# zipnn/zipnn

Measured on AMD Instinct MI355X. Metric: bf16 decompress GB/s (uncompressed bytes / s; compress GB/s beside it), higher is better.
Workload: dtype u8; 1 GPU; 4 GiB synthetic bf16 N(0,0.02) tensor per GPU, 256 KiB chunks, byte-split + huff0 (BASELINE.json configs[1]); chunks_per_gpu=16384, parallelism=chunk-sharded x1, no collectives

## Files before the change

### zipnn_amd/csrc/zn_decode_fused.hip

```cpp
#include "zn_internal.hpp"
#include <atomic>
#include "zn_huf_wave.hpp"
#include "zn_decode_common.hpp"
#include "zn_decode_rest.hpp"

#define ZN_F_THREADS 256
#define ZN_F_RING_BYTES 4096u
#define ZN_F_WAVES_PER_SIMD 4
#define ZN_F_RING_DW (ZN_F_RING_BYTES / 4u)
#define ZN_F_DMAX 6
#define ZN_F_DCAP 4
#define ZN_F_DOM_MAX 154
#define ZN_F_DCONST 4
#define ZN_F_DCONST2 6
#define ZN_F_DENSE_LMIN 4
#define ZN_F_IN_DW (64 * ZN_F_DMAX + 4)
#define ZN_F_TF(D) ((D) * 4 + 1)
#define ZN_F_TLMAX 11u
#define ZN_L16(i) ((i) + (((i) >> 6) << 1))
#define ZN_F_PRIO_SYNC 1
#define ZN_F_PRIO_COUNT 2
#define ZN_F_PRIO_WRITE 3
#if !defined(ZN_SIMT_EMULATOR)
#define ZN_PRIO(v) __builtin_amdgcn_s_setprio(v)
#else
#define ZN_PRIO(v) do { } while (0)
#endif
#if !defined(ZN_SIMT_EMULATOR)
#define ZN_OPAQUE32(x) asm volatile("" : "+v"(x))
#define ZN_KEEP32(x) asm volatile("" :: "v"(x))
__device__ __forceinline__ uint32_t zn_bfi_(uint32_t mask, uint32_t a, uint32_t b) {
  uint32_t d; asm("v_bfi_b32 %0, %1, %2, %3" : "=v"(d) : "s"(mask), "v"(a), "v"(b)); return d;
}
#define ZN_BFI(mask, a, b) zn_bfi_((mask), (a), (b))
#define ZN_NO_IFCVT asm volatile("")
#define ZN_ASM_MARK(txt) asm volatile("; " txt)
#else
#define ZN_NO_IFCVT ((void)0)
#define ZN_ASM_MARK(txt) ((void)0)
#define ZN_OPAQUE32(x) ((void)0)
#define ZN_KEEP32(x) ((void)(x))
#define ZN_BFI(mask, a, b) ((((uint32_t)(a)) & (uint32_t)(mask)) | (((uint32_t)(b)) & ~(uint32_t)(mask)))
#endif
#define ZN_F_DELTA0 44
#define ZN_F_DELTA0_DENSE 88
#define ZN_F_DELTA_FAST 44
#define ZN_F_DELTA_MAX 1024
#define ZN_F_NMIS 3

#if defined(ZN_SIMT_EMULATOR) && defined(ZN_DECODE_HINTED_TU)
extern unsigned long long zn_dbg_tiles[8], zn_dbg_hint[4];
#define ZN_DBG_COUNT(i) do { if (lane == 0) zn_dbg_tiles[i]++; } while (0)
#define ZN_HINT_COUNT(i, n) do { if (lane == 0) zn_dbg_hint[i] += (n); } while (0)
#define ZN_HINT_FIXUP() do { if (hinted && !hfix) { hfix = true; ZN_HINT_COUNT(1, 1); } } while (0)
#elif defined(ZN_SIMT_EMULATOR)
unsigned long long zn_dbg_tiles[8];
extern "C" void zn_debug_tile_counters(unsigned long long* out, int reset) { for (int i = 0; i < 8; i++) { out[i] = zn_dbg_tiles[i]; if (reset) zn_dbg_tiles[i] = 0; } }
#define ZN_DBG_COUNT(i) do { if (lane == 0) zn_dbg_tiles[i]++; } while (0)
unsigned long long zn_dbg_hint[4];
extern "C" void zn_debug_hint_counters(unsigned long long* out, int reset) { for (int i = 0; i < 4; i++) { out[i] = zn_dbg_hint[i]; if (reset) zn_dbg_hint[i] = 0; } }
#define ZN_HINT_COUNT(i, n) do { if (lane == 0) zn_dbg_hint[i] += (n); } while (0)
#define ZN_HINT_FIXUP() do { if (hinted && !hfix) { hfix = true; ZN_HINT_COUNT(1, 1); } } while (0)
#else
#define ZN_DBG_COUNT(i) do { } while (0)
#define ZN_HINT_COUNT(i, n) do { } while (0)
#define ZN_HINT_FIXUP() do { } while (0)
#endif

#define ZN_IN_IDX(i) (i)

#if !defined(ZN_SIMT_EMULATOR)
typedef uint32_t zn_v4u __attribute__((ext_vector_type(4)));
#define ZN_ST128(p, a, b, c, d) __builtin_nontemporal_store((zn_v4u){(a), (b), (c), (d)}, (zn_v4u*)(p))
#else
#define ZN_ST128(p, a, b, c, d) (*(uint4*)(p) = make_uint4((a), (b), (c), (d)))
#endif

#if defined(ZN_SIMT_EMULATOR)
__device__ __forceinline__ uint32_t zn_lane_id() { return threadIdx.x & 63u; }
#else
__device__ __forceinline__ uint32_t zn_lane_id() { return __builtin_amdgcn_mbcnt_hi(~0u, __builtin_amdgcn_mbcnt_lo(~0u, 0u)); }
#endif
__device__ __forceinline__ uint32_t zn_uniform(uint32_t v) { return (uint32_t)__builtin_amdgcn_readfirstlane((int)v); }
__device__ __forceinline__ uint64_t zn_uniform64(uint64_t v) { return ((uint64_t)zn_uniform((uint32_t)(v >> 32)) << 32) | zn_uniform((uint32_t)v); }
template <typename T> __device__ __forceinline__ T* zn_uniform_ptr(T* p) { return ZN_GLOBAL_PTR(T, zn_uniform64((uint64_t)p)); }

typedef uint64_t __attribute__((aligned(1))) zn_u64u;
typedef uint32_t __attribute__((aligned(1))) zn_u32u;
#if !defined(ZN_SIMT_EMULATOR)
#define ZN_LD_RAW32(p) __builtin_nontemporal_load((const zn_u32u*)(p))
#define ZN_LD_RAW64(p) __builtin_nontemporal_load((const zn_u64u*)(p))
#define ZN_LD_STREAM32(p) __builtin_nontemporal_load((const uint32_t*)(p))
#else
#define ZN_LD_RAW32(p) (*(const zn_u32u*)(p))
#define ZN_LD_RAW64(p) (*(const zn_u64u*)(p))
#define ZN_LD_STREAM32(p) (*(const uint32_t*)(p))
#endif
#if defined(ZN_SIMT_EMULATOR)
#define ZN_ST128_4(p, a, b, c, d) (*(uint4*)(p) = make_uint4((a), (b), (c), (d)))
#else
#define ZN_ST128_4(p, a, b, c, d) ZN_ST128(p, a, b, c, d)
#endif

__device__ __forceinline__ uint64_t zn_hint_header_bytes(uint64_t pk) { return ((pk + 1u) * 4u + 63u) & ~63ull; }
__device__ __forceinline__ uint32_t zn_hint_stream_bytes(uint32_t slen, uint32_t seg, uint32_t unit) {
  uint32_t d = ((ZN_F_RING_BYTES - unit - 128u) * slen) / (256u * seg);
  d = d > ZN_F_DCAP ? ZN_F_DCAP : (d < 1u ? 1u : d);
  const uint32_t dw = (slen + 6u) >> 2, td = 64u * d;
  return 64u * ((dw + td - 1u) / td);
}

struct ZnFusedPlane { uint64_t off; uint32_t kind; uint32_t csize; };

struct __attribute__((aligned(16))) ZnFusedLds {
  uint2 lut[1u << ZN_F_TLMAX];
  uint32_t ring[4][ZN_F_RING_DW];
  uint32_t in[4][ZN_F_IN_DW];
  uint8_t symlist[4][256];
  uint32_t rank_start[4][14], sym_start[4][14];
  ZnFusedPlane plane[4][4];
  ZnWaveStats st[4];
  uint32_t what[4];
};

#include "zn_decode_chain.hpp"

template <int NT = ZN_F_THREADS, typename LDS>
__device__ __forceinline__ void zn_fused_fill_luts(LDS& L, uint32_t tid, uint32_t TL, uint32_t j, uint32_t lmin = 1) {
  constexpr int KE = (int)((1u << ZN_F_TLMAX) / (uint32_t)NT);
  uint16_t* lut16 = (uint16_t*)&L.ring[0][0];
  {
    const ZnRankTab rt = zn_load_ranks(L.rank_start[j], L.sym_start[j]);
    for (uint32_t u = tid; u < (1u << TL); u += (uint32_t)NT) lut16[ZN_L16(u)] = (uint16_t)zn_lut_entry(u, TL, L.symlist[j], rt, L.rank_start[j], L.sym_start[j]);
  }
  __syncthreads();
  {
    const uint32_t mask = (1u << TL) - 1u;
    uint32_t pos[KE], cnt[KE], syms[KE], ef[KE];
    for (int k = 0; k < KE; k++) { pos[k] = 0; cnt[k] = 0; syms[k] = 0; ef[k] = 0; }
    const int rounds = (int)zn_uniform(lmin ? (TL / lmin > 4u ? 4u : TL / lmin) : 4u);
    for (int step = 0; step < 4; step++) {
      if (step >= rounds) break;
      for (int k = 0; k < KE; k++) {
        const uint32_t u = tid + (uint32_t)k * (uint32_t)NT;
        if (u <= mask && cnt[k] == (uint32_t)step) {
          const uint32_t e = lut16[ZN_L16((u << pos[k]) & mask)]; const uint32_t len = e >> 8;
          if (pos[k] + len <= TL) {
            if (step > 0) ef[k] |= pos[k] << (16 + 4 * (step - 1));
            syms[k] |= (e & 0xFFu) << (8 * step);
            pos[k] += len; cnt[k]++;
          }
        }
      }
    }
    for (int k = 0; k < KE; k++) {
      const uint32_t u = tid + (uint32_t)k * (uint32_t)NT;
      for (uint32_t i = 1; i <= 3u; i++) if (i >= cnt[k]) ef[k] |= pos[k] << (16u + 4u * (i - 1u));
      if (u <= mask) L.lut[u] = make_uint2(syms[k], ZN_E_META(cnt[k], pos[k], ef[k]));
    }
  }
}

template <int P, int H, int DC, bool X = false, int HM = 0>
__device__ __forceinline__ bool zn_fused_wave(const ZnGeom& g, const uint8_t* __restrict__ body, const uint8_t* body_end,
                                              uint8_t* outq_, const uint8_t* xq_, const ZnFusedPlane (&pl_)[P], const uint8_t* const (&rawq_)[P],
                                              const uint2* lut, uint32_t* ring, uint32_t* in, uint32_t lane_, uint32_t seg_,
                                              uint32_t TL_, uint32_t Du, const uint8_t* stream_, uint32_t slen_, bool ragged ZN_PT_PARAM,
                                              uint8_t* hq_ = nullptr, uint32_t hcap_ = 0) {
  uint32_t lane = lane_;
  uint8_t* const outq = zn_uniform_ptr(outq_); const uint8_t* const xq = zn_uniform_ptr(xq_);
  const uint8_t* const stream = zn_uniform_ptr(stream_);
  const uint32_t seg = zn_uniform(seg_), TL = zn_uniform(TL_), slen = zn_uniform(slen_);
  ZnFusedPlane pl[P]; const uint8_t* rawq[P];
  for (int p = 0; p < P; p++) {
    pl[p].off = zn_uniform64(pl_[p].off); pl[p].kind = zn_uniform(pl_[p].kind); pl[p].csize = zn_uniform(pl_[p].csize);
    rawq[p] = zn_uniform_ptr(rawq_[p]);
  }
  constexpr int EPL = (P == 1) ? 16 : 8;
  constexpr int EW = EPL / 4;
  constexpr uint32_t UNIT = 64u * EPL;
  uint8_t* const hq = HM ? zn_uniform_ptr(hq_) : nullptr; const uint32_t hcap = HM ? zn_uniform(hcap_) : 0u;
  const bool hinted = (HM == 1) && hq != nullptr;
  uint32_t ht = 0, hb_nx = 0;
#define ZN_F_RB4 2
#define ZN_F_SPLIT4 1
  constexpr bool SPLIT = (P == 4) && (ZN_F_SPLIT4 != 0);
#define ZN_F_RB2 3
  constexpr int RB = (P == 2) ? (int)ZN_F_RB2 : (P == 4) ? ZN_F_RB4 : (int)(ZN_F_RING_BYTES / 1024u);
  constexpr int TF = DC ? ZN_F_TF(DC) : 0, TB = 3;
  constexpr bool DENSE = (ZN_F_DCONST2 != 0) && (DC == ZN_F_DCONST2);
  constexpr int UF = DC ? (32 * DC - 31) / 11 : 0;
  ZN_PT_SHARED;

  uint32_t pre[RB][P][EW];
  uint32_t lane_v = lane;
  auto fetch_row_to = [&](uint32_t (&pre)[RB][P][EW], uint32_t first_row_sym, int r) {
    if constexpr (HM == 2) return;
    for (int p = 0; p < P; p++) if (p != H && pl[p].kind == ZN_KIND_RAW) {
      const uint8_t* au = rawq[p] + (first_row_sym + (uint32_t)r * UNIT);
      if constexpr (SPLIT) {
        const uint8_t* a = au + 4u * lane_v;
        pre[r][p][0] = ZN_LD_RAW32(a); pre[r][p][1 % EW] = ZN_LD_RAW32(a + UNIT / 2u);
      } else {
        const uint8_t* a = au + (uint32_t)EPL * lane_v;
        for (int k = 0; k < EW / 2; k++) { const uint64_t t = ZN_LD_RAW64(a + 8 * k); pre[r][p][2 * k] = (uint32_t)t; pre[r][p][2 * k + 1] = (uint32_t)(t >> 32); }
      }
    }
  };
  auto fetch_row = [&](uint32_t first_row_sym, int r) { fetch_row_to(pre, first_row_sym, r); };
  auto fetch_rows = [&](uint32_t first_row_sym, int nrows) {
    for (int r = 0; r < RB; r++) if (r < nrows) fetch_row_to(pre, first_row_sym, r);
  };
  auto emit_rows_from = [&](uint32_t (&pre)[RB][P][EW], bool full_wait, uint32_t first_row_sym, int nrows, uint32_t stage_row0, auto&& after_wait) {
    if (full_wait) __builtin_amdgcn_s_waitcnt(0x0F70);
    ZN_PT(10);
    after_wait();
    constexpr int XW = X ? (P == 4 ? 8 : 4) : 1, XG = 2;
    uint32_t xd[2][XG][XW];
    auto load_delta = [&](int grp) {
      for (int i = 0; i < XG; i++) {
        const int r = grp * XG + i;
        for (int k = 0; k < XW; k++) xd[grp & 1][i][k] = 0;
        if (xq && r < RB && r < nrows) {
          const uint8_t* a = SPLIT ? xq + (uint64_t)(first_row_sym + (uint32_t)r * UNIT) * P + 16u * lane
                                   : xq + (uint64_t)(first_row_sym + (uint32_t)r * UNIT + (uint32_t)EPL * lane) * P;
          for (int k = 0; k < XW / 4; k++) { const uint4 t = *(const uint4*)(a + (SPLIT ? (UNIT / 2u) * P : 16u) * k); xd[grp & 1][i][4 * k] = t.x; xd[grp & 1][i][4 * k + 1] = t.y; xd[grp & 1][i][4 * k + 2] = t.z; xd[grp & 1][i][4 * k + 3] = t.w; }
        }
      }
    };
    if (X) load_delta(0);
    for (int r = 0; r < RB; r++) if (r < nrows) {
      for (int p = 0; p < P; p++) {
        if (p == H) {
          if constexpr (SPLIT) { const uint32_t i = ((stage_row0 + (uint32_t)r) * UNIT >> 2) + lane; for (int k = 0; k < EW; k++) { pre[r][p][k] = ring[i + (UNIT / 8u) * k]; ring[i + (UNIT / 8u) * k] = 0; } }
          else { const uint32_t i = ((stage_row0 + (uint32_t)r) * UNIT + (uint32_t)EPL * lane) >> 2; for (int k = 0; k < EW; k++) { pre[r][p][k] = ring[i + k]; ring[i + k] = 0; } }
        }
        else if (pl[p].kind == ZN_KIND_RLE) { ZN_NO_IFCVT; for (int k = 0; k < EW; k++) pre[r][p][k] = ((uint32_t)pl[p].off & 0xFFu) * 0x01010101u; }
      }
    }
    if (P >= 2 && g.rot) {
      for (int r = 0; r < RB; r++) if (r < nrows)
        for (int k = 0; k < EW; k++) {
          const uint32_t hi = pre[r][P - 1][k], lo = pre[r][(P >= 2) ? P - 2 : 0][k];
          pre[r][P - 1][k] = ZN_BFI(0x80808080u, lo, hi >> 1);
          pre[r][(P >= 2) ? P - 2 : 0][k] = ZN_BFI(0x7F7F7F7Fu, lo, hi << 7);
        }
    }
    if constexpr (HM != 2)
    for (int r = 0; r < RB; r++) if (r < nrows) {
      if (X && r % XG == 0 && r + XG < RB) load_delta(r / XG + 1);
      const uint32_t* xr_ = xd[(r / XG) & 1][r % XG];
      uint8_t* o = (outq + (uint64_t)(first_row_sym + (uint32_t)r * UNIT) * P) + (SPLIT ? 16u : (uint32_t)EPL * (uint32_t)P) * lane_v;
      if (P == 1) {
        if (X) ZN_ST128(o, pre[r][0][0] ^ xr_[0], pre[r][0][1 % EW] ^ xr_[1 % XW], pre[r][0][2 % EW] ^ xr_[2 % XW], pre[r][0][3 % EW] ^ xr_[3 % XW]);
        else ZN_ST128(o, pre[r][0][0], pre[r][0][1 % EW], pre[r][0][2 % EW], pre[r][0][3 % EW]);
      } else if (P == 2) {
        uint32_t x[4];
        x[0] = __builtin_amdgcn_perm(pre[r][1 % P][0], pre[r][0][0], 0x05010400u); x[1] = __builtin_amdgcn_perm(pre[r][1 % P][0], pre[r][0][0], 0x07030602u);
        x[2] = __builtin_amdgcn_perm(pre[r][1 % P][1 % EW], pre[r][0][1 % EW], 0x05010400u); x[3] = __builtin_amdgcn_perm(pre[r][1 % P][1 % EW], pre[r][0][1 % EW], 0x07030602u);
        if (X) for (int k = 0; k < 4; k++) x[k] ^= xr_[k % XW];
        ZN_ST128(o, x[0], x[1], x[2], x[3]);
      } else {
        for (int half = 0; half < 2; half++) {
          const int k = half % EW;
          const uint32_t ab_lo = __builtin_amdgcn_perm(pre[r][1 % P][k], pre[r][0][k], 0x05010400u), ab_hi = __builtin_amdgcn_perm(pre[r][1 % P][k], pre[r][0][k], 0x07030602u);
          const uint32_t cd_lo = __builtin_amdgcn_perm(pre[r][3 % P][k], pre[r][2 % P][k], 0x05010400u), cd_hi = __builtin_amdgcn_perm(pre[r][3 % P][k], pre[r][2 % P][k], 0x07030602u);
          uint32_t x[4];
          x[0] = __builtin_amdgcn_perm(cd_lo, ab_lo, 0x05040100u); x[1] = __builtin_amdgcn_perm(cd_lo, ab_lo, 0x07060302u);
          x[2] = __builtin_amdgcn_perm(cd_hi, ab_hi, 0x05040100u); x[3] = __builtin_amdgcn_perm(cd_hi, ab_hi, 0x07060302u);
          if (X) for (int k = 0; k < 4; k++) x[k] ^= xr_[(4 * half + k) % XW];
          if constexpr (SPLIT) ZN_ST128_4(o + (UNIT / 2u) * P * half, x[0], x[1], x[2], x[3]);
          else *(uint4*)(o + 16 * half) = make_uint4(x[0], x[1], x[2], x[3]);
        }
      }
    }
  };
  auto emit_rows = [&](uint32_t first_row_sym, int nrows, uint32_t stage_row0, auto&& after_wait) { emit_rows_from(pre, true, first_row_sym, nrows, stage_row0, after_wait); };

  uint32_t JF = 0;
  if (H < 0) {
    if constexpr (HM == 2) return true;
    while (JF < seg) {
      const uint32_t left = (seg - JF) / UNIT; const int nr = left < (uint32_t)RB ? (int)left : RB;
      fetch_rows(JF, nr); emit_rows(JF, nr, 0, [] {}); JF += (uint32_t)nr * UNIT;
    }
    ZN_PT(3);
    return true;
  }

  for (uint32_t i = lane; i < ZN_F_RING_DW; i += 64u) ring[i] = 0;
  __builtin_amdgcn_wave_barrier();

  uint32_t J = 0;
  const uint8_t last = stream[slen - 1];
  if (last == 0) return false;
  const uint32_t mis = (uint32_t)((uint64_t)stream & 3u);
  const uint32_t* gdw = (const uint32_t*)(stream - mis);
  const int32_t b0 = (int32_t)(8u * mis);
  int32_t carry = __builtin_amdgcn_readfirstlane(b0 + (int32_t)(8u * (slen - 1u)) + (int32_t)zn_hb32(last));
  int32_t hi_dw = (carry + 31) >> 5;
  const int32_t Di = DC ? DC : (int32_t)Du, TD = 64 * Di;
  int32_t delta = (DENSE ? ZN_F_DELTA0_DENSE : ZN_F_DELTA0) < 32 * Di ? (DENSE ? ZN_F_DELTA0_DENSE : ZN_F_DELTA0) : 32 * Di;
  int nmis = 0;

  uint32_t nx[ZN_F_DMAX], nx_last = 0;
  const int32_t top_dw = hi_dw - 1;
  const bool top_guard = ((const uint8_t*)(gdw + hi_dw) > body_end);
  auto fetch_tile = [&](int32_t lo_dw_, int32_t hi_dw_) {
    const uint32_t* pu = gdw + (lo_dw_ - 1);
    if (lo_dw_ >= 0 && !(top_guard && hi_dw_ - 1 == top_dw)) {
      for (int i = 0; i < ZN_F_DMAX; i++) nx[i] = (i < Di) ? ZN_LD_STREAM32(pu + (lane_v + 64u * (uint32_t)i)) : 0u;
// ... 414 lines not shown
    uint32_t l4 = 0; bool bad = false;
    if (l1 + l2 + l3 + 6u > rem) bad = true; else l4 = rem - 6u - l1 - l2 - l3;
    if (l1 == 0 || l2 == 0 || l3 == 0 || l4 == 0) bad = true;
    __syncthreads();
    if (bad) return -1;
    const uint32_t so = 6u + (wave > 0 ? l1 : 0u) + (wave > 1 ? l2 : 0u) + (wave > 2 ? l3 : 0u);
    const uint8_t* stream2 = js + so; const uint32_t slen2 = (wave == 0) ? l1 : (wave == 1) ? l2 : (wave == 2) ? l3 : l4;
    ZnFusedPlane pl2[P]; const uint8_t* rawq[P];
    for (int p = 0; p < P; p++) { pl2[p] = L.plane[j][p]; rawq[p] = body; if (p != p2) { pl2[p].kind = ZN_KIND_RLE; pl2[p].off = 0; } }
    uint32_t Du2 = ((ZN_F_RING_BYTES - UNIT - 128u) * slen2) / (256u * seg);
    Du2 = Du2 > ZN_F_DMAX ? ZN_F_DMAX : (Du2 < 1u ? 1u : Du2);
    Du2 = (uint32_t)__builtin_amdgcn_readfirstlane((int)Du2);
    ZN_K_HM_MP_REGION
#define ZN_ACC_ARGS g, body, body_end, outq, ZN_K_HM_MP_XQ, pl2, rawq, L.lut, ring, in, lane, seg, TL2, Du2, stream2, slen2, false ZN_PT_PASS ZN_K_HM_MP_HINT_ARGS
    bool ok2;
    if (p2 == 1) ok2 = zn_fused_wave<P, (P >= 2 ? 1 : 0), 0, true ZN_K_HM_MP_TARG>(ZN_ACC_ARGS);
    else if (p2 == 2) ok2 = zn_fused_wave<P, (P >= 4 ? 2 : 0), 0, true ZN_K_HM_MP_TARG>(ZN_ACC_ARGS);
    else ok2 = zn_fused_wave<P, (P >= 4 ? 3 : 0), 0, true ZN_K_HM_MP_TARG>(ZN_ACC_ARGS);
#undef ZN_ACC_ARGS
    ok = ok && ok2;
  }
  return ok ? 1 : 0;
}

static_assert(sizeof(ZnFusedLds) * ZN_F_WAVES_PER_SIMD <= 160u * 1024u, "ZnFusedLds: the LDS budget of ZN_F_WAVES_PER_SIMD workgroups per CU");
template <int P, bool X, bool REST = false ZN_K_HM_TPARAM>
__global__ __launch_bounds__(ZN_F_THREADS, ZN_F_WAVES_PER_SIMD) void ZN_K_DECODE_NAME(ZnSeg one, const ZnSeg* __restrict__ segs, uint32_t nseg,
                                                                  uint8_t* __restrict__ done_all, uint8_t* __restrict__ pdone_all,
                                                                  uint32_t* __restrict__ status, uint32_t ntail,
                                                                  uint8_t* __restrict__ tail_scratch, uint8_t* __restrict__ tail_done, uint32_t only_pending,
                                                                  ZnPlaneDesc* __restrict__ descs_rest, uint32_t nchunk_wg, uint32_t merge_per,
                                                                  uint32_t* __restrict__ tailsync ZN_K_HM_PARAMS) {
  ZN_K_HM_CONST
  constexpr bool RST = REST && !X, INPLACE = REST && X;
  constexpr int EPL = (P == 1) ? 16 : 8;
  constexpr uint32_t UNIT = 64u * EPL;
  __shared__ ZnFusedLds L;

  if (RST && tailsync && blockIdx.x >= ntail + nchunk_wg) {
    const ZnSeg one_c = one;
    zn_tail_merge_wg<P>(L, one_c, segs, nseg, blockIdx.x - (ntail + nchunk_wg), merge_per, tailsync, descs_rest, status, tail_done, tail_scratch);
    return;
  }

  if (blockIdx.x < ntail) {
    const ZnSeg one_c = one; uint32_t tail0 = 0;
    zn_decode_tail_wg(L, one_c, segs, nseg, blockIdx.x, tail_scratch, tail_done, status, &tail0);
    if (RST && tailsync) {
      __syncthreads();
      if (threadIdx.x == 0) { ZN_FLAG_RELEASE(); ZN_FLAG_ADD32(tailsync + 2u * (tail0 / (uint32_t)P), 1u); }
    }
    return;
  }
  const uint32_t wg = blockIdx.x - ntail;
  uint32_t seg_i = 0;
  const ZnSeg S_ = HM ? zn_find_seg<0>(one, segs, nseg, wg, &seg_i) : zn_find_seg<0>(one, segs, nseg, wg);
  ZnSeg S;
  S.g.n = zn_uniform64(S_.g.n); S.g.chunk = zn_uniform64(S_.g.chunk); S.g.K = zn_uniform64(S_.g.K); S.g.P = zn_uniform(S_.g.P); S.g.rot = zn_uniform(S_.g.rot);
  S.body = (const uint8_t*)zn_uniform64((uint64_t)S_.body); S.body_len = zn_uniform64(S_.body_len); S.dst = (uint8_t*)zn_uniform64((uint64_t)S_.dst);
  S.chunk0 = zn_uniform(S_.chunk0); S.desc0 = zn_uniform(S_.desc0); S.wg0 = zn_uniform(S_.wg0); S.ncg = zn_uniform(S_.ncg);
  S.tail0 = zn_uniform(S_.tail0); S.has_tail = zn_uniform(S_.has_tail); S.xr = (const uint8_t*)zn_uniform64((uint64_t)S_.xr);
  const ZnGeom g = S.g;
  const uint8_t* __restrict__ body = ZN_GLOBAL_PTR(const uint8_t, S.body); const uint64_t body_len = S.body_len;
  uint8_t* __restrict__ dst = ZN_GLOBAL_PTR(uint8_t, S.dst); uint8_t* __restrict__ done = done_all + S.chunk0;
  uint8_t* __restrict__ pdone = pdone_all + S.desc0;
#define ZN_REST_CHUNK(c_) do { if constexpr (RST) { \
    static_assert(4u * sizeof(ZnPlanesLds) <= sizeof(ZnFusedLds), "four generic plane decoders fit over the fused kernel's LDS"); \
    __syncthreads(); \
    const ZnSeg one_c_ = one; \
    if (wave < (uint32_t)P) zn_decode_plane_item(reinterpret_cast<ZnPlanesLds*>(&L)[wave], one_c_, segs, nseg, S.desc0 + (uint64_t)wave * g.K + (c_), descs_rest, status, nullptr, lane); \
    __threadfence(); __syncthreads(); \
    for (uint32_t sub_ = 0; sub_ < ZN_MERGE_SUB; sub_++) zn_merge_chunk_item<P>(one_c_, segs, nseg, S.chunk0 + (c_), sub_, descs_rest, nullptr); \
    __syncthreads(); } } while (0)
#define ZN_SET_DONE(c_, v_) do { if (tid == 0) { done[c_] = (v_); if (!(v_)) atomicAdd(status + 1 + (P == 1 ? 0 : P == 2 ? 1 : 2), 1u); } if (tid < (uint32_t)P) pdone[(uint64_t)tid * g.K + (c_)] = (v_); } while (0)
  const uint32_t ncg = S.ncg;
  if (only_pending && zn_uniform(done[(uint64_t)(wg - S.wg0) * ncg]) != 2u) return;

  const uint32_t tid = threadIdx.x, lane = tid & 63u, wave = (uint32_t)__builtin_amdgcn_readfirstlane((int)(tid >> 6));
  const uint64_t c0 = (uint64_t)(wg - S.wg0) * ncg;
  const uint32_t nc = (g.K - c0 < (uint64_t)ncg) ? (uint32_t)(g.K - c0) : ncg;
  const uint32_t plen = (uint32_t)(g.chunk / P);
  const uint32_t seg = plen / 4u;
  const uint8_t* body_end = body + body_len;
  ZN_PT_DECL;

  if (tid < nc * (uint32_t)P) {
    const uint32_t j = tid / (uint32_t)P, p = tid % (uint32_t)P;
    const ZnPcMeta m = zn_pc_meta(g, zn_uniform(S_.kb), zn_uniform(S_.c_lo), body, body_len, p, c0 + j);
    ZnFusedPlane pl; pl.off = m.off; pl.csize = m.csize; pl.kind = 99u;
    if (m.ok && m.type <= 1u && zn_chunk_len(g, c0 + j) == g.chunk) {
      if (m.type == 0u) { if (m.csize >= plen) pl.kind = ZN_KIND_RAW; }
      else if (m.csize == plen) pl.kind = ZN_KIND_RAW;
      else if (m.csize == 1u) { pl.kind = ZN_KIND_RLE; pl.off = body[m.off]; }
      else if (m.csize > 1u && m.csize < plen) pl.kind = ZN_KIND_HUF;
    }
    L.plane[j][p] = pl;
  }
  __syncthreads();
  ZN_PT(0);

  if (wave < nc) {
    int h = -1; uint32_t nhuf = 0;
    bool elig = (g.chunk % (4u * P * UNIT)) == 0 && ((((uint64_t)dst) & 15u) == 0);
    if (X) elig = elig && ((((uint64_t)S.xr) & 15u) == 0);
    for (int p = 0; p < P; p++) {
      const uint32_t kind = L.plane[wave][p].kind;
      if (kind == 99u) elig = false;
      if (kind == ZN_KIND_HUF) { if (h < 0) h = p; nhuf++; }
    }
    (void)nhuf;
    ZnWaveStats st; st.hs = 0; st.nsym = 0; st.tl = 0; st.lmin = 1; st.dom = 0;
    if (elig && h >= 0) {
      const uint32_t csize = L.plane[wave][h].csize;
      uint8_t* scratch = (uint8_t*)&L.ring[wave][0];
      st = zn_wave_read_stats(body + L.plane[wave][h].off, csize, body_end, lane, scratch, L.symlist[wave], L.rank_start[wave],
                              L.sym_start[wave], scratch + 512);
      if (st.hs < 0 || st.tl > ZN_F_TLMAX || (uint32_t)st.hs >= csize || csize - (uint32_t)st.hs < 10u) elig = false;
    }
    if (lane == 0) { L.st[wave] = st; L.what[wave] = elig ? (uint32_t)(h + 2) : 0u; }
  }
  __syncthreads();
  ZN_PT(1);

  for (uint32_t j = 0; j < nc; j++) {
    const uint64_t c = c0 + j;
    if (j > 0) __syncthreads();
    ZN_PT(21);
    const uint32_t what = zn_uniform(L.what[j]);
    if (RST && tailsync && what == 0u && S.has_tail && c == g.K - 1u) {
      if (tid == 0) done[c] = 0; if (tid < (uint32_t)P) pdone[(uint64_t)tid * g.K + c] = 0;
      continue;
    }
    if (what == 0u) { ZN_REST_CHUNK(c); ZN_SET_DONE(c, 0); continue; }
    const int h = (int)what - 2;
    ZnFusedPlane pl[P];
    uint32_t more = 0;
    for (int p = 0; p < P; p++) {
      pl[p].off = zn_uniform64(L.plane[j][p].off); pl[p].kind = zn_uniform(L.plane[j][p].kind); pl[p].csize = zn_uniform(L.plane[j][p].csize);
      if (p > h && h >= 0 && pl[p].kind == ZN_KIND_HUF) { more |= 1u << p; pl[p].kind = ZN_KIND_RLE; pl[p].off = 0; }
    }

    [[maybe_unused]] bool undo = false;
  zn_passes_again:
    uint32_t TL = 0;
    const uint8_t* stream = nullptr; uint32_t slen = 0;
    uint32_t h_before = 0, h_mine = 0;
    bool bad = false;
    if (h >= 0) {
      uint64_t h_off = 0; uint32_t csize = 0;
      for (int p = 0; p < P; p++) if (p == h) { h_off = pl[p].off; csize = pl[p].csize; }
      const uint8_t* src = body + h_off;
      const ZnWaveStats st = L.st[j];
      const int hs = (int)zn_uniform((uint32_t)st.hs); TL = zn_uniform(st.tl);
      zn_fused_fill_luts(L, tid, TL, j, zn_uniform(st.lmin));
      const uint8_t* js = src + hs; const uint32_t rem = csize - (uint32_t)hs;
      const uint32_t l1 = zn_uniform(zn_ld16(js)), l2 = zn_uniform(zn_ld16(js + 2)), l3 = zn_uniform(zn_ld16(js + 4));
      uint32_t l4 = 0;
      if (l1 + l2 + l3 + 6u > rem) bad = true; else l4 = rem - 6u - l1 - l2 - l3;
      if (l1 == 0 || l2 == 0 || l3 == 0 || l4 == 0) bad = true;
      const uint32_t so = 6u + (wave > 0 ? l1 : 0u) + (wave > 1 ? l2 : 0u) + (wave > 2 ? l3 : 0u);
      stream = js + so; slen = (wave == 0) ? l1 : (wave == 1) ? l2 : (wave == 2) ? l3 : l4;
      if constexpr (HM != 0) {
        const uint32_t b1 = zn_hint_stream_bytes(l1, seg, UNIT), b2 = zn_hint_stream_bytes(l2, seg, UNIT), b3 = zn_hint_stream_bytes(l3, seg, UNIT), b4 = zn_hint_stream_bytes(l4, seg, UNIT);
        h_before = (wave > 0 ? b1 : 0u) + (wave > 1 ? b2 : 0u) + (wave > 2 ? b3 : 0u); h_mine = (wave == 0) ? b1 : (wave == 1) ? b2 : (wave == 2) ? b3 : b4;
      }
      __syncthreads();
      ZN_PT(2);
    }
    if (bad) { ZN_REST_CHUNK(c); ZN_SET_DONE(c, 0); continue; }

    const uint8_t* rawq[P];
    for (int p = 0; p < P; p++) rawq[p] = body + pl[p].off + (uint64_t)wave * seg;
    uint8_t* outq = dst + c * g.chunk + (uint64_t)wave * (g.chunk / 4u);
    const uint8_t* xq = (X && S.xr) ? ZN_GLOBAL_PTR(const uint8_t, S.xr) + c * g.chunk + (uint64_t)wave * (g.chunk / 4u) : nullptr;
    uint32_t* ring = L.ring[wave]; uint32_t* in = L.in[wave];
    uint32_t Du = ((ZN_F_RING_BYTES - UNIT - 128u) * slen) / (256u * seg);
    Du = Du > ZN_F_DMAX ? ZN_F_DMAX : (Du < 1u ? 1u : Du);
    const bool dense = ZN_F_DCONST2 && !X && P <= 2 && Du > ZN_F_DCAP && zn_uniform(L.st[j].lmin) >= ZN_F_DENSE_LMIN;
    if (dense) Du = ZN_F_DCONST2;
    else if (ZN_F_DCAP && Du > ZN_F_DCAP && zn_uniform(L.st[j].dom) < ZN_F_DOM_MAX) Du = ZN_F_DCAP;
    Du = (uint32_t)__builtin_amdgcn_readfirstlane((int)Du);
    uint8_t* hq = nullptr; uint32_t hcap = 0;
    if constexpr (HM != 0) {
      ZnHintSeg hs_ = one_h; if (hsegs != nullptr) hs_ = hsegs[seg_i];
      uint8_t* const hbuf = zn_uniform_ptr(hs_.hints); const uint64_t hlen = zn_uniform64(hs_.len);
      const uint64_t kb_ = zn_uniform(S_.kb), ent = ((uint64_t)zn_uniform(S_.c_lo) + c) * (uint32_t)P + (uint32_t)(h < 0 ? 0 : h);
      const uint64_t hdr = zn_hint_header_bytes(kb_ * (uint32_t)P);
      if (h >= 0 && hbuf != nullptr && hlen >= hdr && ent < kb_ * (uint32_t)P) {
        const uint32_t* offs = (const uint32_t*)hbuf;
        const uint32_t o0 = zn_uniform(offs[ent]), o1 = zn_uniform(offs[ent + 1u]);
        if (o0 >= hdr && o1 >= o0 && (uint64_t)o1 <= hlen && (uint64_t)h_before + h_mine <= (uint64_t)(o1 - o0)) { hq = hbuf + o0 + h_before; hcap = h_mine; }
      }
    }
    bool ok;
#define ZN_HINT_ARGS , hq, hcap
#define ZN_WAVE_ARGS g, body, body_end, outq, xq, pl, rawq, L.lut, ring, in, lane, seg, TL, Du, stream, slen, false ZN_PT_PASS
#define ZN_WAVE_CASE(H_) ok = (Du == ZN_F_DCONST) ? zn_fused_wave<P, H_, ZN_F_DCONST, X, HM>(ZN_WAVE_ARGS ZN_HINT_ARGS) \
                            : (dense) ? zn_fused_wave<P, H_, ((X || P > 2 || !ZN_F_DCONST2) ? 0 : ZN_F_DCONST2), X, HM>(ZN_WAVE_ARGS ZN_HINT_ARGS) \
                            : zn_fused_wave<P, H_, 0, X, HM>(ZN_WAVE_ARGS ZN_HINT_ARGS)
    if (h < 0) ok = zn_fused_wave<P, -1, 0, X, HM>(ZN_WAVE_ARGS ZN_HINT_ARGS);
    else if (P == 1 || h == 0) ZN_WAVE_CASE(0);
    else if (P == 2 || h == 1) ZN_WAVE_CASE((P >= 2 ? 1 : 0));
    else if (h == 2) ZN_WAVE_CASE((P >= 4 ? 2 : 0));
    else ZN_WAVE_CASE((P >= 4 ? 3 : 0));
#undef ZN_WAVE_CASE
#undef ZN_WAVE_ARGS
#undef ZN_HINT_ARGS
    if ((HM != 2 || X) && P >= 2 && __builtin_expect(more != 0u, 0)) {
      const int r2 = zn_fused_more_passes<P ZN_K_HM_MP_CALL_TARG>(L, g, body, body_end, outq, j, more, seg ZN_PT_PASS ZN_K_HM_MP_CALL_ARGS);
      if constexpr (INPLACE) {
        if (r2 < 0 && !undo && xq != nullptr && xq == outq) {
          undo = true;
          __syncthreads();
          if (wave == 0) {
            uint8_t* scratch = (uint8_t*)&L.ring[0][0];
            const ZnWaveStats st0 = zn_wave_read_stats(body + L.plane[j][h].off, L.plane[j][h].csize, body_end, lane, scratch, L.symlist[j], L.rank_start[j], L.sym_start[j], scratch + 512);
            if (lane == 0) L.st[j] = st0;
          }
          __syncthreads();
          goto zn_passes_again;
        }
      }
      if (r2 < 0) { ZN_REST_CHUNK(c); ZN_SET_DONE(c, 0); continue; }
      ok = ok && r2 > 0;
    }
    if (!ok) atomicOr(status, ZN_DEV_CORRUPT);
    ZN_SET_DONE(c, 1);
    ZN_PT_COUNT(19, 1);
  }
  ZN_PT_FLUSH();
}

#if defined(ZN_DECODE_HINTED_TU)
__global__ __launch_bounds__(256) void zn_k_hint_size(ZnGeom g, const uint8_t* __restrict__ body, uint64_t body_len, uint32_t* __restrict__ offs, uint64_t* __restrict__ total, uint32_t kind) {
  __shared__ uint32_t sh[256];
  __shared__ uint64_t run;
  const uint32_t tid = threadIdx.x, P = g.P;
  const uint32_t unit = 64u * (P == 1u ? 16u : 8u);
  const uint32_t plen = (uint32_t)(g.chunk / P), seg = plen / 4u;
  const bool geom_ok = (g.chunk % (4ull * P * unit)) == 0;
  const uint8_t* body_end = body + body_len;
  if (tid == 0) run = zn_hint_header_bytes(g.K * P);
  __syncthreads();
  for (uint64_t base = 0; base < g.K; base += 256u) {
    const uint64_t c = base + tid;
    uint32_t sz = 0; uint32_t szp[4] = {0u, 0u, 0u, 0u};
    if (c < g.K && geom_ok && zn_chunk_len(g, c) == g.chunk) {
      bool elig = true; int h = -1; ZnPcMeta mh[4]; bool huf[4] = {false, false, false, false};
      for (uint32_t p = 0; p < P; p++) {
        const ZnPcMeta m = zn_pc_meta(g, (uint32_t)g.K, 0u, body, body_len, p, c);
        uint32_t pk = 99u;
        if (m.ok && m.type <= 1u) {
          if (m.type == 0u) { if (m.csize >= plen) pk = ZN_KIND_RAW; }
          else if (m.csize == plen) pk = ZN_KIND_RAW;
          else if (m.csize == 1u) pk = ZN_KIND_RLE;
          else if (m.csize > 1u && m.csize < plen) pk = ZN_KIND_HUF;
        }
        if (pk == 99u) elig = false;
        mh[p] = m;
        if (pk == ZN_KIND_HUF) { if (h < 0) { h = (int)p; huf[p] = true; } else if (kind != 0u) huf[p] = true; }
      }
      for (uint32_t p = 0; p < P; p++) if (elig && huf[p] && body + mh[p].off + mh[p].csize <= body_end) {
        const uint8_t* src = body + mh[p].off;
        const uint32_t h0 = src[0];
        const uint32_t hs = 1u + (h0 >= 128u ? (h0 - 127u + 1u) / 2u : h0);
        if (hs < mh[p].csize && mh[p].csize - hs >= 10u) {
          const uint8_t* js = src + hs; const uint32_t rem = mh[p].csize - hs;
          const uint32_t l1 = zn_ld16(js), l2 = zn_ld16(js + 2), l3 = zn_ld16(js + 4);
          if (l1 && l2 && l3 && l1 + l2 + l3 + 6u < rem) {
            const uint32_t l4 = rem - 6u - l1 - l2 - l3;
            szp[p] = zn_hint_stream_bytes(l1, seg, unit) + zn_hint_stream_bytes(l2, seg, unit) + zn_hint_stream_bytes(l3, seg, unit) + zn_hint_stream_bytes(l4, seg, unit);
          }
        }
      }
      sz = szp[0] + szp[1] + szp[2] + szp[3];
    }
    sh[tid] = sz;
    __syncthreads();
    for (uint32_t d = 1; d < 256u; d <<= 1) {
      const uint32_t v = (tid >= d) ? sh[tid - d] : 0u;
      __syncthreads();
      sh[tid] += v;
      __syncthreads();
    }
    const uint64_t start = run + (sh[tid] - sz);
    if (offs != nullptr && c < g.K) { uint32_t ahead = 0; for (uint32_t p = 0; p < P; p++) { offs[c * P + p] = (uint32_t)(start + ahead); ahead += szp[p]; } }
    __syncthreads();
    if (tid == 255u) run += sh[255];
    __syncthreads();
  }
  if (tid == 0) { if (offs != nullptr) offs[g.K * P] = (uint32_t)run; *total = run; }
}

void zn_launch_hint_size(const ZnGeom& g, const uint8_t* d_body, uint64_t body_len, uint32_t* d_offs, uint64_t* d_total, hipStream_t stream, int kind) {
  hipLaunchKernelGGL(zn_k_hint_size, dim3(1), dim3(256), 0, stream, g, d_body, body_len, d_offs, d_total, (uint32_t)kind);
  zn_note_kernel("zn_k_hint_size");
}
void zn_launch_decode_hinted(int P, int mode, const ZnSeg& one, const ZnSeg* d_segs, uint32_t nseg, const ZnHintSeg& one_h, const ZnHintSeg* d_hsegs, uint32_t total_wg,
                             uint8_t* d_done, uint8_t* d_pdone, uint32_t* d_status, uint32_t ntail, uint8_t* d_tail_scratch, uint8_t* d_tail_done, hipStream_t stream,
                             bool delta, bool inplace) {
  if (total_wg == 0) return;
  const uint32_t ntail_wg = (mode == 2) ? 0u : 4u * ntail;
#define ZN_GOH(P_, X_, R_, M_) hipLaunchKernelGGL((zn_k_decode_hinted<P_, X_, R_, M_>), dim3(total_wg + ntail_wg), dim3(ZN_F_THREADS), 0, stream, one, d_segs, nseg, d_done, d_pdone, d_status, ntail_wg, d_tail_scratch, d_tail_done, 0u, (ZnPlaneDesc*)nullptr, total_wg, 0u, (uint32_t*)nullptr, one_h, d_hsegs)
  if (!delta) {
    if (mode == 2) { if (P == 1) ZN_GOH(1, false, false, 2); else if (P == 2) ZN_GOH(2, false, false, 2); else ZN_GOH(4, false, false, 2); }
    else { if (P == 1) ZN_GOH(1, false, false, 1); else if (P == 2) ZN_GOH(2, false, false, 1); else ZN_GOH(4, false, false, 1); }
    zn_note_kernel(mode == 2 ? "zn_k_decode_hinted^build" : ntail_wg ? "zn_k_decode_hinted+tail" : "zn_k_decode_hinted");
    return;
  }
  if (mode == 2) { if (P == 1) ZN_GOH(1, true, false, 2); else if (P == 2) ZN_GOH(2, true, false, 2); else ZN_GOH(4, true, false, 2); }
  else if (inplace && P > 1) { if (P == 2) ZN_GOH(2, true, true, 1); else ZN_GOH(4, true, true, 1); }
  else { if (P == 1) ZN_GOH(1, true, false, 1); else if (P == 2) ZN_GOH(2, true, false, 1); else ZN_GOH(4, true, false, 1); }
#undef ZN_GOH
  zn_note_kernel(mode == 2 ? "zn_k_decode_hinted^delta^build" : (inplace && P > 1) ? (ntail_wg ? "zn_k_decode_hinted^delta^inplace+tail" : "zn_k_decode_hinted^delta^inplace")
                                                              : (ntail_wg ? "zn_k_decode_hinted^delta+tail" : "zn_k_decode_hinted^delta"));
}
#endif

#if !defined(ZN_DECODE_HINTED_TU)

#ifdef ZN_PHASE_TIMERS
extern "C" int zn_debug_phase_read(unsigned long long* out, int reset) {
  if (hipDeviceSynchronize() != hipSuccess) return -2;
  if (hipMemcpyFromSymbol(out, HIP_SYMBOL(zn_phase_acc), sizeof(unsigned long long) * 64) != hipSuccess) return -2;
  if (reset) { unsigned long long z[64] = {0}; if (hipMemcpyToSymbol(HIP_SYMBOL(zn_phase_acc), z, sizeof(z)) != hipSuccess) return -2; }
  return 0;
}
#endif

static std::atomic<int> g_zn_decode_group{0};
uint32_t zn_decode_fused_group(uint64_t K) {
  static std::atomic<int> slots_of[64];
  int dev = 0;
  if (hipGetDevice(&dev) != hipSuccess || dev < 0 || dev >= 64) { (void)hipGetLastError(); dev = 0; }
  int slots = slots_of[dev].load(std::memory_order_relaxed);
  if (slots == 0) {
    int cus = 0;
    if (hipDeviceGetAttribute(&cus, hipDeviceAttributeMultiprocessorCount, dev) != hipSuccess || cus <= 0) { (void)hipGetLastError(); cus = 256; }
    slots = cus * ZN_F_WAVES_PER_SIMD;
    slots_of[dev].store(slots, std::memory_order_relaxed);
  }
  uint32_t ncg = 1; uint64_t best = ~0ull;
  for (uint32_t m = 1; m <= 4u; m++) {
    const uint64_t wgs = K ? (K + m - 1u) / m : 1u, rounds = (wgs + (uint64_t)slots - 1u) / (uint64_t)slots;
    const uint64_t cost = rounds * (13u + 85u * m);
    if (cost <= best) { best = cost; ncg = m; }
  }
  const int forced = g_zn_decode_group.load(std::memory_order_relaxed);
  if (forced >= 1 && forced <= 4) ncg = (uint32_t)forced;
  return ncg;
}
static std::atomic<int> g_zn_decode_wide{1};
int zn_decode_use_wide(uint64_t K, bool delta, bool weights_like, uint64_t tail_wgs) {
  const int mode = g_zn_decode_wide.load(std::memory_order_relaxed);
  if (mode == 0 || delta || K == 0) return 0;
  if (mode == 2) return 4;
  if (mode == 3) return 2;
  if (!weights_like) return 0;
  int dev = 0, cus = 0;
  if (hipGetDevice(&dev) != hipSuccess) { (void)hipGetLastError(); return 0; }
  if (hipDeviceGetAttribute(&cus, hipDeviceAttributeMultiprocessorCount, dev) != hipSuccess || cus <= 0) { (void)hipGetLastError(); return 0; }
  return K + tail_wgs <= (uint64_t)cus ? 4 : K + tail_wgs <= 2ull * (uint64_t)cus ? 2 : 0;
}
extern "C" int zn_set_decode_wide(int mode) {
  if (mode < 0 || mode > 3) return -1;
  g_zn_decode_wide.store(mode, std::memory_order_relaxed);
  return 0;
}
extern "C" int zn_decode_group_for(unsigned long long chunks) { return (int)zn_decode_fused_group((uint64_t)chunks); }
extern "C" int zn_set_decode_group(int chunks_per_workgroup) {
  if (chunks_per_workgroup < 0 || chunks_per_workgroup > 4) return -1;
  g_zn_decode_group.store(chunks_per_workgroup, std::memory_order_relaxed);
  return 0;
}

bool zn_launch_decode_fused(int P, const ZnSeg& one, const ZnSeg* d_segs, uint32_t nseg, uint32_t total_wg,
                            uint8_t* d_done, uint8_t* d_pdone, uint32_t* d_status, uint32_t ntail, uint8_t* d_tail_scratch,
                            uint8_t* d_tail_done, bool delta, int wide, bool status_zeroed, ZnPlaneDesc* d_descs_rest, uint32_t* d_tailsync, hipStream_t stream, bool inplace) {
  if (delta || (ntail != 0 && !d_tailsync)) d_descs_rest = nullptr;
  const uint32_t ntt = ntail / (uint32_t)P;
  uint32_t ntail_wg = 4u * ntail;
  uint32_t merge_per = 0;
  if (d_descs_rest && ntail) { merge_per = 32u; while (merge_per > 1u && (uint64_t)merge_per * ntt > 4096u) merge_per >>= 1; }
  else d_tailsync = nullptr;
  const uint32_t nchunk_wg = total_wg;
  if (total_wg == 0) return false;
  const uint32_t only_pending = wide ? 1u : 0u;
  if (wide) {
    const uint32_t zs = (!status_zeroed && ntail == 0) ? 1u : 0u;
#define ZN_GOW(P_, W_) hipLaunchKernelGGL((zn_k_decode_wide<P_, W_>), dim3(total_wg + ntail_wg + merge_per * ntt), dim3(256 * W_), 0, stream, one, d_segs, nseg, d_done, d_pdone, d_status, zs, ntail_wg, d_tail_scratch, d_tail_done, d_tailsync, d_descs_rest, nchunk_wg, merge_per)
    if (wide == 4) { if (P == 1) ZN_GOW(1, 4); else if (P == 2) ZN_GOW(2, 4); else ZN_GOW(4, 4); }
    else { if (P == 1) ZN_GOW(1, 2); else if (P == 2) ZN_GOW(2, 2); else ZN_GOW(4, 2); }
#undef ZN_GOW
    zn_note_kernel(wide == 4 ? (ntail ? (merge_per ? "zn_k_decode_wide+tail+merge" : "zn_k_decode_wide+tail") : "zn_k_decode_wide") : (ntail ? (merge_per ? "zn_k_decode_wide^2+tail+merge" : "zn_k_decode_wide^2+tail") : "zn_k_decode_wide^2"));
    ntail_wg = 0; merge_per = 0; d_tailsync = nullptr;
  }
  total_wg += ntail_wg;
  total_wg += merge_per * ntt;
#define ZN_GO(P_, X_, R_) hipLaunchKernelGGL((zn_k_decode_fused<P_, X_, R_>), dim3(total_wg), dim3(ZN_F_THREADS), 0, stream, one, d_segs, nseg, d_done, d_pdone, d_status, ntail_wg, d_tail_scratch, d_tail_done, only_pending, d_descs_rest, nchunk_wg, merge_per, d_tailsync)
  if (d_descs_rest) { if (P == 1) ZN_GO(1, false, true); else if (P == 2) ZN_GO(2, false, true); else ZN_GO(4, false, true); }
  else if (!delta) { if (P == 1) ZN_GO(1, false, false); else if (P == 2) ZN_GO(2, false, false); else ZN_GO(4, false, false); }
  else if (inplace && P > 1) { if (P == 2) ZN_GO(2, true, true); else ZN_GO(4, true, true); }
  else { if (P == 1) ZN_GO(1, true, false); else if (P == 2) ZN_GO(2, true, false); else ZN_GO(4, true, false); }
#undef ZN_GO
  zn_note_kernel(d_descs_rest ? (ntail && !wide ? "zn_k_decode_fused^rest+tail+merge" : "zn_k_decode_fused^rest") : wide ? "zn_k_decode_fused^pending" : delta ? ((inplace && P > 1) ? (ntail ? "zn_k_decode_fused^delta^inplace+tail" : "zn_k_decode_fused^delta^inplace") : (ntail ? "zn_k_decode_fused^delta+tail" : "zn_k_decode_fused^delta")) : (ntail ? "zn_k_decode_fused+tail" : "zn_k_decode_fused"));
  return d_descs_rest != nullptr;
}
#endif
```

Measured before the change: 2854 GB/s.

## Rewrite Huffman LUT fill with contiguous per-thread cells and branchless multi-symbol pass

The first-level LUT build now gives each thread KE contiguous cells. It finds the code-length bucket by a uniform compare chain instead of the generic rank lookup, and most cells share the first entry, so only short codes are looked up separately. It writes pairs of 16-bit entries as 32-bit stores. The multi-symbol expansion pass becomes branchless, packing count, position and offsets into one register, and removes per-cell divergence. It also adds ASM markers and an emulator-only debug kernel for checking LUT output. The aim is to cut per-chunk LUT setup cost, at the risk of subtle encoding differences in the packed metadata.

```diff
diff --git a/zipnn_amd/csrc/zn_decode_fused.hip b/zipnn_amd/csrc/zn_decode_fused.hip
--- a/zipnn_amd/csrc/zn_decode_fused.hip
+++ b/zipnn_amd/csrc/zn_decode_fused.hip
@@ -128,35 +128,68 @@
 template <int NT = ZN_F_THREADS, typename LDS>
 __device__ __forceinline__ void zn_fused_fill_luts(LDS& L, uint32_t tid, uint32_t TL, uint32_t j, uint32_t lmin = 1) {
   constexpr int KE = (int)((1u << ZN_F_TLMAX) / (uint32_t)NT);
+  constexpr int WF = KE == 8 ? 4 : KE == 4 ? 3 : 2;
+  static_assert(KE == 8 || KE == 4 || KE == 2, "zn_fused_fill_luts: 256, 512 or 1024 threads");
   uint16_t* lut16 = (uint16_t*)&L.ring[0][0];
+  const uint32_t cells = 1u << TL;
   {
-    const ZnRankTab rt = zn_load_ranks(L.rank_start[j], L.sym_start[j]);
-    for (uint32_t u = tid; u < (1u << TL); u += (uint32_t)NT) lut16[ZN_L16(u)] = (uint16_t)zn_lut_entry(u, TL, L.symlist[j], rt, L.rank_start[j], L.sym_start[j]);
+    uint32_t rs[13], bs[13];
+    {
+      uint32_t rv[13], sv[13];
+      for (int w = 1; w <= 12; w++) { rv[w] = L.rank_start[j][w]; sv[w] = L.sym_start[j][w]; }
+      ZN_STEP_FENCE();
+      for (int w = 1; w <= 12; w++) { rs[w] = zn_uniform(rv[w]); bs[w] = zn_uniform(sv[w]) - (rs[w] >> (w - 1)); }
+    }
+    const uint8_t* symlist = L.symlist[j];
+    uint32_t ta = tid; ZN_OPAQUE32(ta);
+    const uint32_t u0 = ta * (uint32_t)KE;
+    uint32_t w = 1, b = bs[1];
+    for (int v = 2; v <= 12; v++) { const bool c = u0 >= rs[v]; w += c ? 1u : 0u; b = c ? bs[v] : b; }
+    const uint32_t e1 = (uint32_t)symlist[((u0 >> (w - 1u)) + b) & 255u] | ((TL + 1u - w) << 8);
+    uint32_t d[KE / 2];
+    for (int i = 0; i < KE / 2; i++) d[i] = e1 | (e1 << 16);
+    if (zn_uniform(tid & ~63u) * (uint32_t)KE < rs[WF]) {
+      if (u0 < rs[WF]) {
+        uint32_t ec[KE], at[KE], wk[KE];
+        for (int k = 0; k < KE; k++) {
+          const uint32_t u = u0 + (uint32_t)k;
+          uint32_t bk = bs[1]; wk[k] = 1;
+          for (int v = 2; v < WF; v++) { const bool c = u >= rs[v]; wk[k] += c ? 1u : 0u; bk = c ? bs[v] : bk; }
+          at[k] = ((u >> (wk[k] - 1u)) + bk) & 255u;
+        }
+        ZN_STEP_FENCE();
+        for (int k = 0; k < KE; k++) ec[k] = (uint32_t)symlist[at[k]];
+        ZN_STEP_FENCE();
+        for (int k = 0; k < KE; k++) ec[k] |= (TL + 1u - wk[k]) << 8;
+        for (int i = 0; i < KE / 2; i++) d[i] = ec[2 * i] | (ec[2 * i + 1] << 16);
+      }
+    }
+    if (u0 < cells) { uint32_t* p = (uint32_t*)&lut16[ZN_L16(u0)]; for (int i = 0; i < KE / 2; i++) p[i] = d[i]; }
   }
   __syncthreads();
   {
-    const uint32_t mask = (1u << TL) - 1u;
-    uint32_t pos[KE], cnt[KE], syms[KE], ef[KE];
-    for (int k = 0; k < KE; k++) { pos[k] = 0; cnt[k] = 0; syms[k] = 0; ef[k] = 0; }
+    const uint32_t mask = cells - 1u;
     const int rounds = (int)zn_uniform(lmin ? (TL / lmin > 4u ? 4u : TL / lmin) : 4u);
+    uint32_t tb = tid; ZN_OPAQUE32(tb);
+    uint32_t m[KE], syms[KE];
+    for (int k = 0; k < KE; k++) { m[k] = 0; syms[k] = 0; }
+#pragma unroll
     for (int step = 0; step < 4; step++) {
-      if (step >= rounds) break;
-      for (int k = 0; k < KE; k++) {
-        const uint32_t u = tid + (uint32_t)k * (uint32_t)NT;
-        if (u <= mask && cnt[k] == (uint32_t)step) {
-          const uint32_t e = lut16[ZN_L16((u << pos[k]) & mask)]; const uint32_t len = e >> 8;
-          if (pos[k] + len <= TL) {
-            if (step > 0) ef[k] |= pos[k] << (16 + 4 * (step - 1));
-            syms[k] |= (e & 0xFFu) << (8 * step);
-            pos[k] += len; cnt[k]++;
-          }
+      if (step < rounds) {
+        uint32_t e[KE];
+        for (int k = 0; k < KE; k++) e[k] = lut16[ZN_L16(((tb + (uint32_t)k * (uint32_t)NT) << (m[k] & 15u)) & mask)];
+        for (int k = 0; k < KE; k++) {
+          const uint32_t len = e[k] >> 8;
+          const bool fit = (m[k] & 15u) + len <= TL;
+          m[k] += fit ? (len | 0x100u) : 0u;
+          syms[k] |= (fit ? (e[k] & 0xFFu) : 0u) << (8 * step);
         }
       }
+      if (step < 3) for (int k = 0; k < KE; k++) m[k] |= (m[k] & 15u) << (16 + 4 * step);
     }
     for (int k = 0; k < KE; k++) {
-      const uint32_t u = tid + (uint32_t)k * (uint32_t)NT;
-      for (uint32_t i = 1; i <= 3u; i++) if (i >= cnt[k]) ef[k] |= pos[k] << (16u + 4u * (i - 1u));
-      if (u <= mask) L.lut[u] = make_uint2(syms[k], ZN_E_META(cnt[k], pos[k], ef[k]));
+      const uint32_t u = tb + (uint32_t)k * (uint32_t)NT;
+      if (u <= mask) L.lut[u] = make_uint2(syms[k], m[k]);
     }
   }
 }
@@ -877,7 +910,9 @@
       const uint8_t* src = body + h_off;
       const ZnWaveStats st = L.st[j];
       const int hs = (int)zn_uniform((uint32_t)st.hs); TL = zn_uniform(st.tl);
+      ZN_ASM_MARK("ZN_MARK lutfill");
       zn_fused_fill_luts(L, tid, TL, j, zn_uniform(st.lmin));
+      ZN_ASM_MARK("ZN_MARK lutfill_end");
       const uint8_t* js = src + hs; const uint32_t rem = csize - (uint32_t)hs;
       const uint32_t l1 = zn_uniform(zn_ld16(js)), l2 = zn_uniform(zn_ld16(js + 2)), l3 = zn_uniform(zn_ld16(js + 4));
       uint32_t l4 = 0;
@@ -1044,6 +1079,38 @@
 
 #if !defined(ZN_DECODE_HINTED_TU)
 
+#if defined(ZN_SIMT_EMULATOR)
+template <int NT, typename LDS>
+__global__ void zn_k_debug_lut_fill(const uint8_t* symlist, const uint32_t* rs, const uint32_t* ss, uint32_t TL, uint32_t lmin, uint2* out) {
+  __shared__ LDS L;
+  const uint32_t tid = threadIdx.x;
+  for (uint32_t i = tid; i < 256u; i += (uint32_t)NT) L.symlist[0][i] = symlist[i];
+  if (tid < 14u) { L.rank_start[0][tid] = rs[tid]; L.sym_start[0][tid] = ss[tid]; }
+  for (uint32_t i = tid; i < (1u << ZN_F_TLMAX); i += (uint32_t)NT) L.lut[i] = make_uint2(0xDEADBEEFu, 0xDEADBEEFu);
+  __syncthreads();
+  zn_fused_fill_luts<NT>(L, tid, TL, 0, lmin);
+  __syncthreads();
+  for (uint32_t u = tid; u < (1u << ZN_F_TLMAX); u += (uint32_t)NT) out[u] = L.lut[u];
+}
+extern "C" int zn_debug_lut_fill(const uint8_t* weights, uint32_t TL, uint32_t lmin, uint32_t nthreads, uint2* out ) {
+  if (TL < 1u || TL > ZN_F_TLMAX) return -1;
+  uint32_t cnt[13] = {0}, rs[14], ss[14], cells = 0, syms = 0;
+  for (int s = 0; s < 256; s++) { if (weights[s] > 12u || weights[s] > TL) return -1; cnt[weights[s]]++; }
+  rs[0] = 0; ss[0] = 0;
+  for (uint32_t v = 1; v <= 12; v++) { rs[v] = cells; ss[v] = syms; cells += cnt[v] << (v - 1u); syms += cnt[v]; }
+  rs[13] = cells; ss[13] = syms;
+  if (cells != (1u << TL)) return -1;
+  uint8_t symlist[256] = {0}; uint32_t at[13];
+  for (uint32_t v = 1; v <= 12; v++) at[v] = ss[v];
+  for (int s = 0; s < 256; s++) if (weights[s]) symlist[at[weights[s]]++] = (uint8_t)s;
+  if (nthreads == 256u) hipLaunchKernelGGL((zn_k_debug_lut_fill<256, ZnFusedLds>), dim3(1), dim3(256), 0, 0, symlist, rs, ss, TL, lmin, out);
+  else if (nthreads == 512u) hipLaunchKernelGGL((zn_k_debug_lut_fill<512, ZnWideLds<2>>), dim3(1), dim3(512), 0, 0, symlist, rs, ss, TL, lmin, out);
+  else if (nthreads == 1024u) hipLaunchKernelGGL((zn_k_debug_lut_fill<1024, ZnWideLds<4>>), dim3(1), dim3(1024), 0, 0, symlist, rs, ss, TL, lmin, out);
+  else return -1;
+  return 0;
+}
+#endif
+
 #ifdef ZN_PHASE_TIMERS
 extern "C" int zn_debug_phase_read(unsigned long long* out, int reset) {
   if (hipDeviceSynchronize() != hipSuccess) return -2;
```

Result: no change. 2882 GB/s, median of 6 (+1.0%).
